# gmweir/PYFFT

Measured on AMD Instinct MI355X. Metric: Msamples/sec Welch-PSD 4096-pt Hann 50% overlap, complex64, higher is better.
Workload: dtype f32

## Files before the change

### pyfft_amd/csrc/k_welch_pipe.hip

```cpp
#include "launch.h"
#include <type_traits>
#define SP_PIPE_AHEAD 2
namespace sp {

template <bool CPLX, int SHIFT, int MODE>
__global__ __launch_bounds__(768) void k_welch_pipe(const void *__restrict__ x_in, const float *__restrict__ win,
                                                     int64_t nframes, int64_t fpg, float *__restrict__ trend_in, XfTables tb,
                                                     float *__restrict__ partial, cf *__restrict__ spartial, int64_t x_cs, int gpr) {
    constexpr int N = 4096;
    constexpr bool RP = MODE >= 3 && MODE != 8 && MODE != 9;
    constexpr bool ONEPASS = MODE == 1 || MODE == 4 || MODE == 7 || MODE == 8 || MODE == 9, COG = MODE == 2 || MODE == 8;
    constexpr bool LOBE = MODE == 9;
    constexpr bool SPEC = MODE == 5 || MODE == 7;
    const void *x = SPEC ? (const void *)(reinterpret_cast<const float *>(x_in) + (int64_t)blockIdx.y * x_cs) : x_in;
    float *trend = SPEC ? trend_in + 4 * blockIdx.y : trend_in;
    static_assert(!RP || (!CPLX && SHIFT == 8), "the real-pair form is for real input at hop = nfft / 2");
    using PL = FftPlan<N>;
    using F = WgFft<N>;
    constexpr int T = PL::T, R = PL::R, KEEP = R - SHIFT, IMG = F::IMG0, IMGB = PL::LDS_ELEMS;
    static_assert(T == 256 && R == 16 && PL::NP == 3, "three radix-16 passes over 256 threads");
    extern __shared__ __attribute__((aligned(16))) unsigned char smem_raw[];
    cf *smem = reinterpret_cast<cf *>(smem_raw);
    cf *imgA = smem, *imgB = smem + 2 * IMG;
    const int role = __builtin_amdgcn_readfirstlane((int)threadIdx.x >> 8);
    const int tid = (int)threadIdx.x & 255;
    const int hop = SHIFT * T;

    cf mu;
    if constexpr (ONEPASS) {
        const int64_t span = (nframes - 1) * (int64_t)hop + N;
        const int64_t pitch = span / 16;
        constexpr int NU = SPEC ? 4 : 1, NTH = SPEC ? 3 * T : T, NWV = SPEC ? 12 : 4;
        const int lt = SPEC ? (int)threadIdx.x : tid;
        float sx = 0.f, sy = 0.f;
#pragma unroll
        for (int r = 0; r < 16; ++r)
#pragma unroll
            for (int u = 0; u < NU; ++u) {
                int64_t i = pitch * r + (int64_t)(lt + NTH * u);
                i = i < span ? i : span - 1;
                const cf v = load_sample(x, i, CPLX);
                sx += v.x;
                sy += v.y;
            }
        sx = wave_sum64(sx);
        sy = wave_sum64(sy);
        float *red = reinterpret_cast<float *>(smem);
        if ((SPEC || role == 0) && (tid & 63) == 0) {
            red[2 * (lt >> 6)] = sx;
            red[2 * (lt >> 6) + 1] = sy;
        }
        __syncthreads();
        double tx = 0.0, ty = 0.0;
#pragma unroll
        for (int wv = 0; wv < NWV; ++wv) {
            tx += (double)red[2 * wv];
            ty += (double)red[2 * wv + 1];
        }
        mu = mk((float)(tx / (16.0 * NTH * NU)), (float)(ty / (16.0 * NTH * NU)));
        __syncthreads();
        if (blockIdx.x == 0 && threadIdx.x == 0) {
            trend[0] = mu.x;
            trend[1] = mu.y;
            trend[2] = 0.f;
            trend[3] = 0.f;
        }
    } else {
        mu = load_trend(trend).m;
    }
    const int64_t gid = blockIdx.x;
    const int64_t g0 = gid * fpg;
    const int64_t last = nframes - 1;
    int64_t trips = (RP ? (nframes + 1) / 2 : nframes) - g0;
    trips = trips < 0 ? 0 : (trips > fpg ? fpg : trips);
    constexpr int DRAIN = 4;
    const int64_t periods = trips + DRAIN;
    F f;
    constexpr bool UPROT = !RP;
    float tau_out[16];
    if constexpr (UPROT) {
        if (role == 0) f.template load_tau_out<0>(tb.tw, tid, tau_out);
        else if (role == 1) f.template load_tau_out<1>(tb.tw, tid, tau_out);
    }

    if (role == 0 && RP) {
        const float *xr = reinterpret_cast<const float *>(x);
        float m = mu.x;
        asm volatile("" : "+v"(m));
        float w[R], sacc[SHIFT];
#pragma unroll
        for (int t = 0; t < R; ++t) w[t] = win[tid + T * t];
#pragma unroll
        for (int s = 0; s < SHIFT; ++s) sacc[s] = 0.f;
        auto issue_chunk = [&](float (&dst)[R], int64_t q) __attribute__((always_inline)) {
            const int64_t q1 = 2 * q <= nframes ? q : 0, q2 = 2 * q + 1 <= nframes ? q : 0;
            const float *b1 = xr + q1 * (int64_t)N, *b2 = xr + q2 * (int64_t)N;
#pragma unroll
            for (int t = 0; t < R; ++t) {
                const unsigned off = (unsigned)(tid + T * t);
                dst[t] = __builtin_nontemporal_load((t < R / 2 ? b1 : b2) + off);
            }
        };
        float ca[R], cb[R], cc[R];
        issue_chunk(ca, g0);
        issue_chunk(cb, g0 + 1);
#pragma unroll
        for (int t = 0; t < R; ++t) {
            ca[t] -= m;
            cb[t] -= m;
        }
        auto frame = [&](auto hb, int64_t i, cf *img, float (&cur)[R], float (&nxt)[R], float (&fill)[R]) __attribute__((always_inline)) {
            constexpr bool HB = decltype(hb)::value;
            issue_chunk(fill, g0 + i + 2);
            __builtin_amdgcn_sched_barrier(0);
            cf v[R];
            if constexpr (!ONEPASS) {
#pragma unroll
                for (int t = 0; t < R; ++t) v[t] = mk(cur[t], HB ? (t < R / 2 ? cur[t + R / 2] : nxt[t - R / 2]) : 0.f);
                if constexpr (UPROT) f.bfly_scatter_win_rot(v, w, tau_out, img, tid);
                else f.bfly_scatter_win(v, w, img, tid);
            } else {
#pragma unroll
                for (int t = 0; t < R; ++t) v[t] = mk(w[t] * cur[t], HB ? w[t] * (t < R / 2 ? cur[t + R / 2] : nxt[t - R / 2]) : 0.f);
                if constexpr (UPROT) f.template bfly_scatter_rot<0, false>(v, tau_out, img, tid);
                else f.template bfly_scatter<0>(v, img, tid);
            }
            __builtin_amdgcn_sched_barrier(0);
            if constexpr (ONEPASS) {
#pragma unroll
                for (int s = 0; s < SHIFT; ++s) sacc[s] += HB ? cur[R / 2 + s] + nxt[s] : cur[R / 2 + s];
            }
#pragma unroll
            for (int t = 0; t < R; ++t) fill[t] -= m;
        };
        const std::true_type yes;
        const std::false_type no;
        int64_t i = 0;
        for (; i + 6 < trips; i += 6) {
            frame(yes, i, imgA, ca, cb, cc);
            __syncthreads();
            frame(yes, i + 1, imgA + IMG, cb, cc, ca);
            __syncthreads();
            frame(yes, i + 2, imgA, cc, ca, cb);
            __syncthreads();
            frame(yes, i + 3, imgA + IMG, ca, cb, cc);
            __syncthreads();
            frame(yes, i + 4, imgA, cb, cc, ca);
            __syncthreads();
            frame(yes, i + 5, imgA + IMG, cc, ca, cb);
            __syncthreads();
        }
        for (; i < trips; ++i) {
            cf *img = (i & 1) ? imgA + IMG : imgA;
            const bool has_b = 2 * (g0 + i) + 1 < nframes;
            if (has_b) {
                if (i % 3 == 0) frame(yes, i, img, ca, cb, cc);
                else if (i % 3 == 1) frame(yes, i, img, cb, cc, ca);
                else frame(yes, i, img, cc, ca, cb);
            } else {
                if (i % 3 == 0) frame(no, i, img, ca, cb, cc);
                else if (i % 3 == 1) frame(no, i, img, cb, cc, ca);
                else frame(no, i, img, cc, ca, cb);
            }
            __syncthreads();
        }
#pragma unroll
        for (int d = 0; d < DRAIN; ++d) __syncthreads();
        if constexpr (ONEPASS) {
#pragma unroll
            for (int s = 0; s < SHIFT; ++s)
                spartial[((SPEC ? (int64_t)blockIdx.y * gridDim.x : 0) + gid) * hop + tid + T * s] = mk(sacc[s], 0.f);
        }
    } else if (role == 0) {
        asm volatile("" : "+v"(mu.x), "+v"(mu.y));
        float w[R];
        cf sacc[SHIFT], raw[R];
#pragma unroll
        for (int t = 0; t < R; ++t) w[t] = win[tid + T * t];
#pragma unroll
        for (int s = 0; s < SHIFT; ++s) sacc[s] = mk(0.f, 0.f);
        {
            const int64_t base = (g0 < nframes ? g0 : last) * hop + tid;
#pragma unroll
            for (int t = 0; t < R; ++t) raw[t] = load_sample(x, base + T * t, CPLX) - mu;
        }
        auto issue_part = [&](cf (&dst)[SHIFT], int64_t q, int s0, int s1) __attribute__((always_inline)) {
            const int64_t gq = g0 + q;
            const int64_t gn = gq < nframes ? gq : last;
            const int64_t ubase = gn * hop + (int64_t)T * KEEP;
#pragma unroll
            for (int s = s0; s < s1; ++s) {
                const unsigned off = (unsigned)(tid + T * s);
                if (CPLX) {
                    const sp_f2v r = __builtin_nontemporal_load(reinterpret_cast<const sp_f2v *>(x) + ubase + off);
                    dst[s] = mk(r.x, r.y);
                } else {
                    dst[s] = mk(__builtin_nontemporal_load(reinterpret_cast<const float *>(x) + ubase + off), 0.f);
                }
            }
        };
        auto issue = [&](cf (&dst)[SHIFT], int64_t q) __attribute__((always_inline)) { issue_part(dst, q, 0, SHIFT); };
        constexpr int AHEAD = (SP_PIPE_AHEAD >= 2 && SHIFT <= 8) ? (SP_PIPE_AHEAD >= 3 ? 3 : 2) : 1;
        constexpr bool SPREAD = AHEAD >= 2;
        auto frame = [&](int64_t i, cf *img, cf (&fill)[SHIFT], cf (&take)[SHIFT]) __attribute__((always_inline)) {
            if constexpr (SPREAD) issue_part(fill, i + AHEAD, 0, SHIFT / 4);
            else issue(fill, i + AHEAD);
            __builtin_amdgcn_sched_barrier(0);
            cf v[R];
            constexpr bool WINFOLD = SPREAD;
#pragma unroll
            for (int t = 0; t < R; ++t) v[t] = WINFOLD ? raw[t] : w[t] * raw[t];
            if constexpr (SPREAD) {
            {
                auto store = [&](int k, cf val) __attribute__((always_inline)) {
                    img[F::template phys<0>(tid * 16 + k)] = UPROT ? rot_tan(val, tau_out[k]) : val;
                    if (k >= 12 && k < 15) issue_part(fill, i + AHEAD, (k - 11) * (SHIFT / 4), (k - 10) * (SHIFT / 4));
                };
                if constexpr (WINFOLD) dft16s_es_win(v, w, store);
                else dft16s_es<false>(v, f.t16[0], store);
            }
            } else {
            if constexpr (UPROT) f.template bfly_scatter_rot<0, false>(v, tau_out, img, tid);
            else f.template bfly_scatter<0>(v, img, tid);
            }
            __builtin_amdgcn_sched_barrier(0);
#pragma unroll
            for (int s = 0; s < SHIFT; ++s)
                if constexpr (ONEPASS && !LOBE) sacc[s] = sacc[s] + raw[KEEP + s];
#pragma unroll
            for (int t = 0; t < KEEP; ++t) raw[t] = raw[t + SHIFT];
#pragma unroll
            for (int s = 0; s < SHIFT; ++s) raw[KEEP + s] = take[s] - mu;
        };
        int64_t i = 0;
        if constexpr (AHEAD == 3) {
            cf s0[SHIFT], s1[SHIFT], s2[SHIFT];
            issue(s1, 1);
            issue(s2, 2);
            for (; i + 2 < trips; i += 3) {
                frame(i, (i & 1) ? imgA + IMG : imgA, s0, s1);
                __syncthreads();
                frame(i + 1, ((i + 1) & 1) ? imgA + IMG : imgA, s1, s2);
                __syncthreads();
                frame(i + 2, ((i + 2) & 1) ? imgA + IMG : imgA, s2, s0);
                __syncthreads();
            }
            for (; i < trips; ++i) {
                cf *img = (i & 1) ? imgA + IMG : imgA;
                if (i % 3 == 0) frame(i, img, s0, s1);
                else if (i % 3 == 1) frame(i, img, s1, s2);
                else frame(i, img, s2, s0);
                __syncthreads();
            }
        } else if constexpr (AHEAD == 2) {
            cf nxa[SHIFT], nxb[SHIFT];
            issue(nxa, 1);
            for (; i + 1 < trips; i += 2) {
                frame(i, imgA, nxb, nxa);
                __syncthreads();
                frame(i + 1, imgA + IMG, nxa, nxb);
                __syncthreads();
            }
            if (i < trips) {
                frame(i, imgA, nxb, nxa);
                __syncthreads();
            }
        } else {
            for (; i + 1 < trips; i += 2) {
                cf nx0[SHIFT], nx1[SHIFT];
                frame(i, imgA, nx0, nx0);
                __syncthreads();
                frame(i + 1, imgA + IMG, nx1, nx1);
                __syncthreads();
            }
            if (i < trips) {
                cf nx0[SHIFT];
                frame(i, imgA, nx0, nx0);
                __syncthreads();
            }
        }
#pragma unroll
        for (int d = 0; d < DRAIN; ++d) __syncthreads();
#pragma unroll
        for (int s = 0; s < SHIFT; ++s)
            if constexpr (ONEPASS && !LOBE) spartial[gid * hop + tid + T * s] = sacc[s];
    } else if (role == 1) {
        f.template load_tw_one<1>(tb.tw, tid);
        cf va[R], vb[R];
        auto step = [&](auto steady, cf (&fill)[R], cf (&use)[R], int64_t p, const cf *src, cf *dst) __attribute__((always_inline)) {
            constexpr bool STEADY = decltype(steady)::value;
            if (STEADY || (p >= 1 && p <= trips)) f.template gather<0>(fill, src, tid);
            if (STEADY || (p >= 2 && p <= trips + 1)) {
                if constexpr (UPROT) f.template bfly_scatter_rot<1, true>(use, tau_out, dst, tid);
                else f.template bfly_scatter<1>(use, dst, tid);
            }
            __syncthreads();
            if constexpr (STEADY) __builtin_amdgcn_sched_barrier(0);
        };
        const std::true_type yes;
        const std::false_type no;
        step(no, va, vb, 0, imgA + IMG, imgB);
        step(no, vb, va, 1, imgA, imgB + IMGB);
        int64_t p = 2;
        for (; p + 1 <= trips; p += 2) {
            step(yes, va, vb, p, imgA + IMG, imgB);
            step(yes, vb, va, p + 1, imgA, imgB + IMGB);
        }
        for (; p < periods; p += 2) {
            step(no, va, vb, p, imgA + IMG, imgB);
            if (p + 1 < periods) step(no, vb, va, p + 1, imgA, imgB + IMGB);
        }
    } else {
        f.template load_tw_one<2>(tb.tw, tid);
        float acc[R];
#pragma unroll
        for (int t = 0; t < R; ++t) acc[t] = 0.f;
        cf bs_lo = mk(0.f, 0.f), bs_hi = mk(0.f, 0.f);
        const unsigned zlo = (unsigned)((tid >> 3) * 512 + (tid & 7));
        cf held[SPEC ? R : 1];
        cf va[R], vb[R];
        cf pend = mk(0.f, 0.f);
        auto flush = [&](int64_t i) __attribute__((always_inline)) {
            const int sel = (int)(i & 63), li = tid & 63;
            const int64_t gg = g0 + (i - sel) + li;
            if (li <= sel && gg < nframes) reinterpret_cast<cf *>(partial)[(int64_t)(tid >> 6) * nframes + gg] = pend;
        };
        auto step = [&](auto steady, cf (&fill)[R], cf (&use)[R], int64_t p, const cf *src) __attribute__((always_inline)) {
            constexpr bool STEADY = decltype(steady)::value;
            if (STEADY || (p >= 3 && p <= trips + 2)) {
                f.template gather<1>(fill, src, tid);
            }
            if (STEADY || (p >= 4 && p <= trips + 3)) {
                if constexpr (UPROT) f.template bfly_prerot<2>(use, tid);
                else f.template bfly<2>(use, tid);
                if constexpr (SPEC) {
                    const int64_t pr = g0 + (p - 4);
                    const bool lone = (pr & 1) == 0 && p == trips + 3;
                    if ((pr & 1) == 0 && !lone) {
#pragma unroll
                        for (int t = 0; t < R; ++t) held[t] = use[t];
                    } else {
                        float4 *zb = reinterpret_cast<float4 *>(partial) + ((pr >> 1) * (int64_t)gpr * 512 + (int64_t)blockIdx.y * 8);
                        unsigned bl = zlo;
                        asm volatile("" : "+v"(bl));
#pragma unroll
                        for (int t = 0; t < R; ++t) {
                            const float4 q = lone ? make_float4(use[t].x, use[t].y, 0.f, 0.f)
                                                  : make_float4(held[t].x, held[t].y, use[t].x, use[t].y);
                            st_stream(zb + (bl + 16384u * t), q);
                        }
                    }
                } else if constexpr (COG) {
                    if constexpr (MODE == 8) {
                        const int64_t gf = g0 + (p - 4);
                        cf *lobe = reinterpret_cast<cf *>(partial) + 4 * nframes + gf * 8;
                        if (gf < nframes) {
                            if (tid <= 3) lobe[3 + tid] = use[0];
                            if (tid >= T - 3) lobe[3 - (T - tid)] = use[R - 1];
                        }
                    }
                    float numc = 0.f, den = 0.f;
#pragma unroll
                    for (int t = 0; t < R; ++t) {
                        const float pw = cnorm(use[t]);
                        numc = fmaf(pw, (float)(T * t - (t >= R / 2 ? N : 0)), numc);
                        den += pw;
                    }
                    float num = fmaf((float)tid, den, numc);
                    num = wave_sum64(num);
                    den = wave_sum64(den);
                    const int64_t i = p - 4;
                    if ((tid & 63) == (int)(i & 63)) pend = mk(num, den);
                    if ((i & 63) == 63 || i == trips - 1) flush(i);
                } else {
#pragma unroll
                    for (int t = 0; t < R; ++t) acc[t] = fmaf(use[t].y, use[t].y, fmaf(use[t].x, use[t].x, acc[t]));
                    if constexpr (LOBE) {
                        bs_lo = bs_lo + use[0];
                        bs_hi = bs_hi + use[R - 1];
                    }
                }
            }
            __syncthreads();
            if constexpr (STEADY) __builtin_amdgcn_sched_barrier(0);
        };
        const std::true_type yes;
        const std::false_type no;
        int64_t p = 0;
#pragma unroll 1
        for (; p < DRAIN; p += 2) {
            step(no, va, vb, p, imgB + IMGB);
            step(no, vb, va, p + 1, imgB);
        }
        for (; p + 1 <= trips + 2; p += 2) {
            step(yes, va, vb, p, imgB + IMGB);
            step(yes, vb, va, p + 1, imgB);
        }
        for (; p < periods; p += 2) {
            step(no, va, vb, p, imgB + IMGB);
            if (p + 1 < periods) step(no, vb, va, p + 1, imgB);
        }
        if constexpr (!COG && !SPEC) {
#pragma unroll
            for (int t = 0; t < R; ++t) partial[gid * N + tid + T * t] = acc[t];
            if constexpr (LOBE) {
                if (tid <= 3) spartial[gid * 8 + 3 + tid] = bs_lo;
                if (tid >= T - 3) spartial[gid * 8 + 3 - (T - tid)] = bs_hi;
                if (tid == 4) spartial[gid * 8 + 7] = mk(0.f, 0.f);
            }
        }
    }
}

bool welch_pipe_eligible(const Xf &xf, int hop) {
    return !xf.blue && xf.L == 4096 && (hop == 2048 || hop == 1024 || hop == 4096);
}

int launch_welch_pipe(LaunchCtx c, const void *x, bool cplx, const float *win, int hop, int64_t nframes, float *trend,
                      const Xf &xf, float *partial, const RunPart &rp, cf *spartial, int mode, int nch, int64_t x_cs, int gpr) {
    const size_t lds = sizeof(cf) * 4 * (size_t)FftPlan<4096>::LDS_ELEMS;
#define PIPE_(CP, S, OP)                                                                                  \
    {                                                                                                 \
        if (lds_raise<k_welch_pipe<CP, S, OP>>(lds)) return -1;                                       \
        if (c.stop)                                                                                   \
            hipExtLaunchKernelGGL((k_welch_pipe<CP, S, OP>), dim3(rp.blocks, gy), dim3(768), lds, c.stream, nullptr, c.stop, 0, x, win, \
                                  nframes, rp.fpg, trend, xf.tb, partial, spartial, x_cs, gpr);       \
        else                                                                                          \
            hipLaunchKernelGGL((k_welch_pipe<CP, S, OP>), dim3(rp.blocks, gy), dim3(768), lds, c.stream, x, win, nframes, rp.fpg, trend, \
                               xf.tb, partial, spartial, x_cs, gpr);                                  \
    }
    const int shift = hop / 256;
    const unsigned gy = mode == 5 ? (unsigned)nch : 1u;
#define PIPE_S_(CP, OP)                                                                               \
    if (shift == 8) PIPE_(CP, 8, OP) else if (shift == 4) PIPE_(CP, 4, OP) else PIPE_(CP, 16, OP)
    if (mode == 5) {
        if (cplx || shift != 8 || nch < 1 || gpr < 1) return -1;
        if (spartial) PIPE_(false, 8, 7) else PIPE_(false, 8, 5)
    } else if (mode == 3) {
        if (cplx || shift != 8) return -1;
        if (spartial) PIPE_(false, 8, 4) else PIPE_(false, 8, 3)
    } else if (mode == 2 && spartial) {
        if (shift == 8) { if (cplx) PIPE_(true, 8, 8) else PIPE_(false, 8, 8) }
        else if (shift == 4) { if (cplx) PIPE_(true, 4, 8) else PIPE_(false, 4, 8) }
        else return -1;
    } else if (mode == 2) {
        if (cplx) { PIPE_S_(true, 2) } else { PIPE_S_(false, 2) }
    } else if (mode == 9) {
        if (!spartial || shift == 16) return -1;
        if (shift == 8) { if (cplx) PIPE_(true, 8, 9) else PIPE_(false, 8, 9) }
        else { if (cplx) PIPE_(true, 4, 9) else PIPE_(false, 4, 9) }
    } else if (spartial) {
        if (cplx) { PIPE_S_(true, 1) } else { PIPE_S_(false, 1) }
    } else {
        if (cplx) { PIPE_S_(true, 0) } else { PIPE_S_(false, 0) }
    }
#undef PIPE_S_
#undef PIPE_
    return 0;
}

}
```

### pyfft_amd/csrc/launch.h

```cpp
#pragma once
#include <limits.h>
#include <stdlib.h>
#include "kernels.h"
#include "nufft_plan.h"
#include "ar_plan.h"
#include "sub_plan.h"
#include "dwt_plan.h"
#include <hip/hip_runtime.h>
#include <hip/hip_ext.h>

namespace sp {

inline bool env_flag(const char *name) {
    const char *v = getenv(name);
    return v && v[0] && v[0] != '0';
}
inline int env_int(const char *name, int dflt) {
    const char *v = getenv(name);
    return v ? atoi(v) : dflt;
}

struct LaunchCtx {
    hipStream_t stream;
    int ncu;
    hipEvent_t stop = nullptr;
};

struct Xf {
    XfTables tb;
    int L;
    bool blue;
};

constexpr int fpw_of(int L) {
    const int R = L < 16 ? L : 16, T = L / R, WG = T >= 256 ? T : 256;
    return WG / T;
}
constexpr size_t xf_image_bytes(int L, int nbuf = 1) { return (size_t)fpw_of(L) * (size_t)(L + 16) * 8 * nbuf; }
template <int L> constexpr bool xf_image_agrees() {
    if constexpr (L < 8192) {
        if (!xf_image_agrees<2 * L>()) return false;
    }
    return WgCfg<L>::FPW == fpw_of(L) && WgCfg<L>::lds_bytes(1) == xf_image_bytes(L) && WgCfg<L>::lds_bytes(2) == xf_image_bytes(L, 2);
}
static_assert(xf_image_agrees<32>(), "fpw_of and xf_image_bytes are the kernels' FPW and lds_bytes at every L of 32 .. 8192");

#define SP_LDS_MAX ((size_t)160 * 1024)
template <auto K> int lds_raise(size_t lds_bytes) {
    static size_t raised = 64 * 1024;
    if (lds_bytes <= raised) return 0;
    if (lds_bytes > SP_LDS_MAX ||
        hipFuncSetAttribute((const void *)K, hipFuncAttributeMaxDynamicSharedMemorySize, (int)SP_LDS_MAX) != hipSuccess)
        return -1;
    raised = SP_LDS_MAX;
    return 0;
}

template <class X> struct XfTag {
    using type = X;
};
template <int LO, int HI, class F> int for_pow2(int L, F f) {
    if (L == LO) return f(XfTag<XfPow2<LO>>{});
    if constexpr (LO < HI) return for_pow2<2 * LO, HI>(L, f);
    else return -1;
}

inline bool runs_cover(int64_t n, int64_t per, int64_t runs) {
    return runs >= 1 && runs <= 0x7fffffff && (runs - 1) * per < n && runs * per >= n;
}
inline bool band_in_transform(bool cplx, int L, int b0, int nb) {
    return nb >= 1 && b0 >= 0 && b0 < L && nb <= L && (cplx || b0 + nb <= L / 2 + 1);
}

struct RunPart {
    int64_t groups, fpg;
    int blocks;
};
inline RunPart run_partition(int L, int64_t nframes, int ncu, int groups_per_cu = 0) {
    if (groups_per_cu <= 0) groups_per_cu = 4;
    const int fpw = fpw_of(L);
    const int64_t target = (int64_t)ncu * groups_per_cu * fpw;
    int64_t f = (nframes + target - 1) / target;
    if (f < 1) f = 1;
    const int64_t G = (nframes + f - 1) / f;
    RunPart r;
    r.fpg = f;
    r.blocks = (int)((G + fpw - 1) / fpw);
    r.groups = (int64_t)r.blocks * fpw;
    return r;
}
inline RunPart run_partition_2d(int L, int64_t nframes, int ncu, int ny, int64_t slots = 0) {
    const int fpw = fpw_of(L);
    int64_t target = ((int64_t)ncu * 8 + ny - 1) / (ny > 0 ? ny : 1) * fpw;
    if (target < 8 * fpw) target = 8 * fpw;
    int64_t f = (nframes + target - 1) / target;
    if (f < 1) f = 1;
    if (slots > 0 && ny > 0) {
        const int64_t wg = ((nframes + f - 1) / f + fpw - 1) / fpw * ny;
        int64_t rounds = (wg + slots / 2) / slots;
        if (rounds < 1) rounds = 1;
        const int64_t groups = rounds * slots / ny * fpw;
        if (groups >= 1) {
            const int64_t f2 = (nframes + groups - 1) / groups;
            if (f2 >= 1 && f2 <= 4 * f) f = f2;
        }
    }
    const int64_t G = (nframes + f - 1) / f;
    RunPart r;
    r.fpg = f;
    r.blocks = (int)((G + fpw - 1) / fpw);
    r.groups = (int64_t)r.blocks * fpw;
    return r;
}
inline int strided_blocks(int L, int64_t items, int ncu, int per_cu = 4) {
    const int fpw = fpw_of(L);
    int64_t b = (items + fpw - 1) / fpw;
    int64_t cap = (int64_t)ncu * (L >= 4096 ? per_cu : 16);
    if (L == 2048) {
        const int64_t q = b / 4;
        if (q < cap) cap = q > (int64_t)ncu * 2 ? q : (int64_t)ncu * 2;
    }
    if (b > cap) b = cap;
    if (b < 1) b = 1;
    return (int)b;
}

int resident_per_cu(const void *fn, int threads, size_t lds_bytes);
int welch_rp_groups_per_cu(const Xf &xf, bool lin);
int csd_pair_resident(const Xf &xf, bool lin, bool onepass);
int stft_rp_groups_per_cu(const Xf &xf, bool lin, int hop, int sided, int out_power, bool pseg);

int launch_fft_c2c(LaunchCtx c, const cf *in, cf *out, int64_t batch, int inverse, const Xf &xf,
                   BigTw bt = BigTw{nullptr, nullptr, 0, 0});
int launch_fft_cols(LaunchCtx c, const cf *in, cf *out, int64_t ncols, int64_t nouter, int64_t es, int64_t os, int64_t twmul,
                    int conj_in, const Xf &xf, BigTw bt, int64_t hmask_n = 0,
                    ColsIn ci = ColsIn{0, nullptr, nullptr, nullptr, 0}, int tw_outer = 0);
int launch_fft_rows_rev(LaunchCtx c, const cf *in, cf *out, int64_t A, int64_t B, int conj_out, float scale, const Xf &xf,
                        RowsOut ro = RowsOut{nullptr, 0, 0, nullptr});
int launch_transpose_c(LaunchCtx c, const cf *in, cf *out, int64_t rows, int64_t cols, int conj, float scale, int64_t batch = 1);
int launch_pack_real(LaunchCtx c, const float *x, int64_t n_in, const double *mean, int64_t L, cf *out);
int launch_cmul_vec(LaunchCtx c, const cf *a, const cf *b, int64_t n, int conj_out, cf *out, int64_t batch = 1);
int launch_blue_pre(LaunchCtx c, const cf *in, const cf *chirp, int64_t n, int64_t L, int conj_in, cf *out, int64_t batch = 1);
int launch_blue_post(LaunchCtx c, const cf *in, const cf *chirp, int64_t n, int conj_out, float scale, cf *out, int64_t batch = 1,
                     int64_t in_ld = 0);
int launch_hilbert_mask(LaunchCtx c, cf *X, int64_t n);
int launch_xc_pack(LaunchCtx c, const float *x1, const float *x2, int64_t n, int64_t L, const double *mom, cf *z);
int launch_xc_mid(LaunchCtx c, const cf *Z, int64_t L, cf *R);
int launch_xc_mid_half(LaunchCtx c, const cf *Z, int64_t L, BigTw bt, cf *Zp);
int launch_xc_out(LaunchCtx c, const cf *r, int64_t n, int64_t L, const double *mom, float *co);
bool welch_carry_eligible(const Xf &xf, int hop, bool lin);
int launch_welch(LaunchCtx c, const void *x, bool cplx, const float *win, int hop, int64_t nframes, const float *trend,
                 bool lin, const Xf &xf, float *partial, const RunPart &rp, bool allow_carry, cf *spartial,
                 const char **kname, int segmean = 0);
bool welch_pipe_eligible(const Xf &xf, int hop);
int launch_welch_pipe(LaunchCtx c, const void *x, bool cplx, const float *win, int hop, int64_t nframes, float *trend,
                      const Xf &xf, float *partial, const RunPart &rp, cf *spartial, int mode = 0, int nch = 1, int64_t x_cs = 0,
                      int gpr = 0);
int launch_op_estimate(LaunchCtx c, const void *x, bool cplx, int64_t nsig, double *part, float *trend);
int launch_op_reduce(LaunchCtx c, const void *x, bool cplx, const float *trend, const float *partial, const cf *spartial,
                     int64_t G, const Xf &xf, int hop, int64_t nframes, int64_t nmean, OnePass st, double *sum_out);
int launch_op_finish(LaunchCtx c, const void *x, bool cplx, const float *trend, const float *win, OnePass st,
                     const double *mean_in, int64_t nmean, const Xf &xf, int hop, int64_t nframes, cf *cw, const cf *Wf,
                     int sided, double scale, double *out, bool export_state = false);
int launch_op_apply(LaunchCtx c, const double *state, const cf *Wf, int n, int sided, double scale, double *out,
                    const double *mean = nullptr);
int opx_tot_blocks();
int launch_welch_opx(LaunchCtx c, const void *x, bool cplx, bool pair, const float *win, int hop, int64_t nframes,
                     const float *trend, const Xf &xf, const RunPart &rp, float *partial, cf *cpart);
int launch_opx_reduce(LaunchCtx c, const float *partial, const cf *cpart, int64_t G, const Xf &xf, const void *x, bool cplx,
                      const float *trend, int hop, int64_t nframes, int64_t nmean, double *A, double *csum, double *tpart);
int launch_opx_finish(LaunchCtx c, const float *win, const double *A, const double *csum, const double *tpart, const float *trend,
                      int hop, int64_t nframes, int64_t nmean, bool sym, const Xf &xf, double *out);
int launch_op_fused(LaunchCtx c, const void *x, bool cplx, const float *trend, const float *win, const float *partial,
                    const cf *spartial, int64_t G, int n, int hop, int64_t nframes, int64_t nmean, OnePass st, unsigned *ticket,
                    CogLobe lb, const double *mean_in, int sided, double scale, double *out, bool export_state,
                    OpPrev prev = OpPrev{nullptr, nullptr, nullptr, 0, 0.0}, bool light = false, double cola_c = 0.0);
int launch_welch_finish(LaunchCtx c, const float *partial, int64_t G, const Xf &xf, int sided, double scale, double *out,
                        int sym = 0);
int launch_welch_rp(LaunchCtx c, const float *x, const float *win, int hop, int64_t nframes, const float *trend, bool lin,
                    const Xf &xf, float *partial, const RunPart &rp);
int launch_stft_rp(LaunchCtx c, const float *x, const float *win, int hop, int64_t nframes, const float *trend, bool lin,
                   const Xf &xf, const RunPart &rp, int sided, float amp, int out_power, void *out, double *pseg,
                   int nchan = 1, int64_t x_cs = 0, int64_t out_cs = 0, int out_ld = 0);
int launch_csd(LaunchCtx c, const void *x, const void *y, bool cplx, int nch, int64_t y_ld, const float *win, int hop,
               int64_t nframes, const float *trend_x, const float *trend_y, bool lin, const Xf &xf, float *partial,
               const RunPart &rp, int segmean = 0);
int launch_csd_finish(LaunchCtx c, const float *partial, int64_t G, const Xf &xf, int nch, int sided, double scale,
                      double *pxx, double *pyy, double *pxy);
int launch_stft(LaunchCtx c, const void *x, bool cplx, const float *win, int hop, int64_t nframes, const float *trend,
                bool lin, const Xf &xf, const RunPart &rp, int sided, float amp, int out_power, void *out, double *pseg, int segmean = 0,
                cf *cog = nullptr, int klo = 0, int khi = 0);
int launch_cog_finish(LaunchCtx c, const cf *acc, int wpf, int64_t nframes, double df, double *out);
int launch_cog_carry(LaunchCtx c, const void *x, bool cplx, const float *win, int hop, int64_t nframes, const float *trend,
                     const Xf &xf, cf *cog, const RunPart &rp, int klo, int khi);
bool csd_rp_eligible(const Xf &xf);
int launch_csd_rp(LaunchCtx c, const float *x, const float *y, int nch, int64_t y_ld, const float *win, int hop,
                  int64_t nframes, const float *trend_x, const float *trend_y, bool lin, const Xf &xf, float *partial,
                  const RunPart &rp);
int launch_csd_rp_finish(LaunchCtx c, const float *partial, int64_t G, const Xf &xf, int nch, int sided, double scale,
                         double *pxx, double *pyy, double *pxy);
int launch_pairspec(LaunchCtx c, const float *x, const float *win, int hop, int64_t nframes, const float *trend, bool lin,
                    const Xf &xf, const RunPart &rp, cf *Zx);
int launch_csd_pair(LaunchCtx c, const float *y, int nch, int64_t y_ld, const float *win, int hop, int64_t nframes,
                    float *trend_y, bool lin, const Xf &xf, const cf *Zx, float *partial, const RunPart &rp, cf *spartial = nullptr);
int launch_csd_pair_finish(LaunchCtx c, const float *partial, int64_t G, const Xf &xf, int nch, int sided, double scale,
                           double *pyy, double *pxy, const double *st_y = nullptr, const double *st_x = nullptr, const cf *Wf = nullptr,
                           const float *trend_x = nullptr, const float *trend_y = nullptr, int64_t nmean = 0, int64_t M = 0);
#define SP_COLSUM_SLICES 256
int launch_colsum_real(LaunchCtx c, const float *x, const float *trend, int H, int64_t M, cf *out);
int launch_csdm_finish(LaunchCtx c, double *G, int nch, int nb, double scale);
int launch_csdm_transpose_kgc(LaunchCtx c, const cf *Xs, cf *Xt, int nch, int nchp, int64_t m, int64_t mp, int nb);
int launch_csdm_mfma(LaunchCtx c, const cf *Xt, int nch, int nchp, int64_t mp, int nb, double *G);
int launch_csdm_bf16(LaunchCtx c, const cf *Xs, cf *Xt_tail, int nch, int64_t m, int nb, double *G, int ld, int two_pieces = 0, int init = 0);
int launch_csdm_fold(LaunchCtx c, const double *H, double *G, int nch, int n, const double *st = nullptr, const cf *Wf = nullptr,
                     const float *trend = nullptr, int64_t nmean = 0, int64_t M = 0, double scale = 1.0, int init = 0);
int launch_cm_blocksums(LaunchCtx c, const cf *spartial, int nch, int runs, int hop, double *Sl);
int launch_op_finish_channels(LaunchCtx c, const void *x, int64_t x_cs, int nch, const float *trend, const float *win,
                              const double *Sl, const cf *Wf, int hop, int64_t nframes, int64_t nmean, const Xf &xf, double *out,
                              bool cplx = false);
int launch_cog_finish_op(LaunchCtx c, const cf *acc, int wpf, int64_t nframes, double df, double *out, const cf *lobe, CogLobe lb,
                         const double *st, const float *trend, int64_t nmean, int n);
int launch_csdm_fused(LaunchCtx c, const cf *Xs, cf *Xt_tail, int nch, int64_t m, int nb, double *G, int ld = 0);
int launch_hilbert_mid(LaunchCtx c, cf *Z, int64_t M, BigTw bt);
int launch_hilbert_rowsmid(LaunchCtx c, cf *Tm, int64_t A, int64_t B, const Xf &xc, BigTw btN, const cf *tw2c);
int launch_xc_rowsmid(LaunchCtx c, cf *Tm, int64_t A, int64_t B, const Xf &xc, const Xf &xc2, BigTw btL, BigTw btM);
int launch_fft_cols_lag(LaunchCtx c, const cf *in, int64_t ncols, int64_t nouter, int64_t es, int64_t os, const Xf &xf, RowsOut ro);
int launch_fft_cols_inv(LaunchCtx c, const cf *in, cf *out, int64_t ncols, int64_t nouter, int64_t es, int64_t os, int64_t twmul,
                        const Xf &xf, BigTw bt, float scale, const RowsOut *analytic);
int launch_hilbert(LaunchCtx c, const float *x, int64_t n_in, int64_t x_ld, int64_t batch, const Xf &xf, cf *out,
                   const cf *H = nullptr);
int launch_spec_mul(LaunchCtx c, cf *X, const cf *H, int64_t n);
int frame_sum_slices(int ncu, int nch, int nfft, int64_t nframes);
int launch_frame_sum(LaunchCtx c, const void *x, bool cplx, int64_t x_ld, int nch, int nfft, int hop, int64_t nframes,
                     const float *trend, bool lin, double *out, double *part);
int launch_fftfilt(LaunchCtx c, const float *x, int64_t n, int ntaps, const cf *Hs, const Xf &xf, float *y);
int launch_xcorr(LaunchCtx c, const float *x1, const float *x2, int64_t n, const double *mom, const Xf &xf, float *co);
int launch_moments(LaunchCtx c, const void *x, bool cplx, int64_t n, int mode, double *partial_scratch, double *out_d,
// ... 768 lines not shown
```

### pyfft_amd/csrc/spectral.hip

```cpp
#include "../../include/spectral.h"
#include "../../include/spectral_ext.h"
#include "../../include/spectral_tfr.h"
#include "../../include/spectral_quad.h"
#include "../../include/spectral_cyclo.h"
#include "../../include/spectral_uneven.h"
#include "../../include/spectral_wbic.h"
#include "../../include/spectral_fam.h"
#include "../../include/spectral_nufft.h"
#include "../../include/spectral_nufft2.h"
#include "../../include/spectral_ar.h"
#include "../../include/spectral_sub.h"
#include "../../include/spectral_dwt.h"
#include "launch.h"
#include "stage.h"
#include "table_cache.h"

#include <hip/hip_runtime.h>
#include <rccl/rccl.h>
#include <dlfcn.h>
#include <limits.h>
#include <math.h>
#include <stdarg.h>
#include <stdio.h>
#include <stdlib.h>
#include <string.h>

#include <map>
#include <mutex>
#include <string>
#include <vector>

using namespace sp;

#define SP_VERSION 110
#define SP_MAX_WG_FFT 8192
#define SP_MAX_BIG_LOG2 26

namespace {

thread_local std::string g_err;

int fail(const char *fmt, ...) {
    char buf[512];
    va_list ap;
    va_start(ap, fmt);
    vsnprintf(buf, sizeof buf, fmt, ap);
    va_end(ap);
    g_err = buf;
    return -1;
}

#define HIPCHK(expr)                                                                                  \
    do {                                                                                              \
        hipError_t e_ = (expr);                                                                       \
        if (e_ != hipSuccess) return fail("%s failed: %s (%s:%d)", #expr, hipGetErrorString(e_), __FILE__, __LINE__); \
    } while (0)
#define LAUNCHCHK(expr)                                                                               \
    do {                                                                                              \
        if ((expr) != 0) return fail("%s: no kernel instantiated for this transform length (%s:%d)", #expr, __FILE__, __LINE__); \
        HIPCHK(hipGetLastError());                                                                    \
    } while (0)

struct Scratch {
    void *p = nullptr;
    size_t cap = 0;
    int ensure(size_t bytes) {
        if (bytes <= cap) return 0;
        if (p) (void)hipFree(p);
        p = nullptr;
        cap = 0;
        size_t want = bytes + (bytes >> 3) + 4096;
        if (hipMalloc(&p, want) != hipSuccess) return fail("hipMalloc(%zu) failed", want);
        cap = want;
        return 0;
    }
    void release() {
        if (p) (void)hipFree(p);
        p = nullptr;
        cap = 0;
    }
};

struct BlueTab {
    cf *chirp, *bf;
    int L;
};

struct Ctx {
    bool ready = false;
    int device = 0;
    int ncu = 256;
    hipStream_t stream = nullptr;
    std::map<int64_t, cf *> twiddles;
    std::map<int64_t, BlueTab> blue;
    Scratch in0, in1, out0, work, small, trends, onepass, ticket, epi;
    Scratch pend_trend;
    Scratch bigA, bigB, bigT, blueA, blueB, longrec;
    Scratch sosY, sosZ;
    Scratch bsIn, bsS, bsP, bsA;
    Scratch mtS;
    Scratch wbW, wbP, wbA;
    Scratch famZ, famA;
    Scratch nuRec, nuGrid;
    Scratch subPart, subMat;
    Scratch dwtS;
    Scratch arPart, arSmall;
    Scratch cmS, cmT, cmG, cmH, cmO;
    std::map<int64_t, BigTw> bigtw;
    std::map<int64_t, BlueTab> blue_big;
    std::mutex mu;
    bool profile = false, prof_valid = false;
    hipEvent_t ev0 = nullptr, ev1 = nullptr, ev_sw = nullptr;
    const char *last_kernel = "";
} g;

LaunchCtx lc() { return LaunchCtx{g.stream, g.ncu}; }

struct Pending {
    bool valid = false;
    const void *xd = nullptr;
    bool cplx = false;
    int64_t nsig = 0, nframes = 0, nmean = 0;
    int nfft = 0, hop = 0;
    Xf xf;
    const float *win_d = nullptr;
    const cf *Wf = nullptr;
    OnePass st;
    float *trend_f = nullptr;
    cf *cw = nullptr;
    double *sum_d = nullptr;
    double *state = nullptr;
} g_pend;

struct ProfScope {
    bool on;
    hipStream_t st;
    explicit ProfScope(hipStream_t s = nullptr) : on(g.profile), st(s ? s : g.stream) {
        if (on) (void)hipEventRecord(g.ev0, st);
    }
    ~ProfScope() {
        if (on) {
            (void)hipEventRecord(g.ev1, st);
            g.prof_valid = true;
        }
    }
};

int ensure_init() {
    if (g.ready) return 0;
    return sp_init(-1);
}

bool is_pow2(int64_t n) { return n >= 1 && (n & (n - 1)) == 0; }
int64_t next_pow2(int64_t n) {
    int64_t p = 1;
    while (p < n) p <<= 1;
    return p;
}

int get_twiddles(int64_t n, const cf **out) {
    auto it = g.twiddles.find(n);
    if (it != g.twiddles.end()) {
        *out = it->second;
        return 0;
    }
    std::vector<cf> h((size_t)n);
    for (int64_t m = 0; m < n; ++m) {
        const double a = -2.0 * M_PI * (double)m / (double)n;
        h[(size_t)m] = make_float2((float)cos(a), (float)sin(a));
    }
    cf *d = nullptr;
    HIPCHK(hipMalloc((void **)&d, sizeof(cf) * (size_t)n));
    HIPCHK(hipMemcpy(d, h.data(), sizeof(cf) * (size_t)n, hipMemcpyHostToDevice));
    g.twiddles[n] = d;
    *out = d;
    return 0;
}

int get_xf(int64_t n, Xf *xf) {
    if (n < 2) return fail("transform length %lld too short", (long long)n);
    if (is_pow2(n) && n <= SP_MAX_WG_FFT) {
        xf->L = (int)n;
        xf->blue = false;
        xf->tb.n = (int)n;
        xf->tb.chirp = xf->tb.bf = nullptr;
        return get_twiddles(n, &xf->tb.tw);
    }
    int64_t L = next_pow2(2 * n - 1);
    if (L < 16) L = 16;
    if (L > SP_MAX_WG_FFT)
        return fail("transform length %lld not supported yet (powers of two up to %d, other lengths up to %d)",
                    (long long)n, SP_MAX_WG_FFT, SP_MAX_WG_FFT / 2);
    xf->L = (int)L;
    xf->blue = true;
    xf->tb.n = (int)n;
    if (get_twiddles(L, &xf->tb.tw)) return -1;
    auto it = g.blue.find(n);
    if (it == g.blue.end()) {
        std::vector<cf> ch((size_t)n), bw((size_t)L, make_float2(0.f, 0.f));
        for (int64_t m = 0; m < n; ++m) {
            const int64_t q = (m * m) % (2 * n);
            const double a = M_PI * (double)q / (double)n;
            ch[(size_t)m] = make_float2((float)cos(a), (float)-sin(a));
            const cf b = make_float2((float)(cos(a) / (double)L), (float)(sin(a) / (double)L));
            bw[(size_t)m] = b;
            if (m > 0) bw[(size_t)(L - m)] = b;
        }
        BlueTab t;
        t.L = (int)L;
        HIPCHK(hipMalloc((void **)&t.chirp, sizeof(cf) * (size_t)n));
        HIPCHK(hipMalloc((void **)&t.bf, sizeof(cf) * (size_t)L));
        HIPCHK(hipMemcpy(t.chirp, ch.data(), sizeof(cf) * (size_t)n, hipMemcpyHostToDevice));
        HIPCHK(hipMemcpy(t.bf, bw.data(), sizeof(cf) * (size_t)L, hipMemcpyHostToDevice));
        Xf p2;
        if (get_xf(L, &p2)) return -1;
        LAUNCHCHK(launch_fft_c2c(lc(), t.bf, t.bf, 1, 0, p2));
        HIPCHK(hipStreamSynchronize(g.stream));
        g.blue[n] = t;
        it = g.blue.find(n);
    }
    xf->tb.chirp = it->second.chirp;
    xf->tb.bf = it->second.bf;
    return 0;
}

TableCache g_tables;

int g_passes[10] = {0, 0, 0, 0, 0, 0, 0, 0, 0, 0};
inline void note_slices(int64_t n) {
    if (n > g_passes[1]) g_passes[1] = (int)n;
}
inline int64_t hook_cap(const char *name, int64_t v) {
    const int64_t h = env_int(name, 0);
    return h > 0 && h < v ? h : v;
}

struct ApiLock {
    std::lock_guard<std::mutex> lk;
    ApiLock() : lk(g.mu) {
        g_tables.begin_call();
        g_passes[0] = g_passes[1] = g_passes[2] = g_passes[3] = g_passes[4] = g_passes[5] = g_passes[6] = g_passes[7] = g_passes[8] = g_passes[9] = 0;
    }
};

struct Stage {
    const bool host;
    int done = 0;
    StagePlan plan;
    explicit Stage(int mem) : host(!mem) {}
    template <class H, class D> void in(Scratch &s, const H *h, size_t bytes, const D **dev) {
        *dev = (const D *)h;
        if (host) plan.add(&s, h, nullptr, bytes, dev);
    }
    template <class H, class D> void out(Scratch &s, H *h, size_t bytes, D **dev) {
        *dev = (D *)h;
        if (host) plan.add(&s, nullptr, h, bytes, dev);
    }
    template <class H, class D> void inout(Scratch &s, const H *h_in, H *h_out, size_t bytes, const D **din, D **dout) {
        *din = (const D *)h_in;
        *dout = (D *)h_out;
        if (host) plan.add(&s, h_in, h_out, bytes, dout, din);
    }
    int commit() {
        if (!host) return 0;
        if (plan.err) return fail("staging: %s", plan.err);
        for (int a = 0; a < plan.nareas; ++a)
            if (!plan.area[a].sealed) {
                if (((Scratch *)plan.area[a].key)->ensure(plan.area[a].total)) return -1;
                plan.seal(a);
// ... 889 lines not shown
    geng.epi = nullptr;
    geng.nsub = 0;
}

int engine_apply_locked(int s) {
    EngineSlot &sl = geng.slot[s];
    const int nfft = (int)sl.win.size();
    Xf xf;
    if (get_xf(nfft, &xf)) return -1;
    void *Wf_d;
    if (get_window_spectrum(sl.win.data(), nfft, xf, &Wf_d)) return -1;
    LAUNCHCHK(launch_op_apply(LaunchCtx{geng.epi, g.ncu}, (const double *)geng.st[s].p, (const cf *)Wf_d, nfft, sl.sided,
                              sl.scale / (double)sl.frames_total, sl.out));
    return 0;
}

bool welch_generic_shape(int nfft, int hop) {
    if (!wg_capable(nfft)) return false;
    Xf xf;
    if (get_xf(nfft, &xf)) return false;
    return !welch_carry_eligible(xf, hop, false);
}

int welch_export_locked(const void *xd, bool cplx, int64_t nsig, const float *win, int nfft, int hop, int64_t nframes,
                        int64_t nmean, double *st_d, const OpPrev *prev = nullptr, hipEvent_t prev_wait = nullptr,
                        bool *prev_done = nullptr, const SplitLaunch *sl = nullptr) {
    FusedOut fo{true, SP_SIDED_RAW, 1.0, st_d, false};
    if (prev) {
        fo.prev = *prev;
        fo.prev_wait = prev_wait;
    }
    if (welch_accum_locked(xd, cplx, nsig, win, nfft, hop, nframes, nmean, false, &fo, sl)) return -1;
    g_pend.valid = false;
    if (prev_done) *prev_done = fo.prev_done;
    if (fo.done) return 0;
    LAUNCHCHK(launch_op_finish(sl ? LaunchCtx{sl->epi, g.ncu} : lc(), g_pend.xd, g_pend.cplx, g_pend.trend_f, g_pend.win_d, g_pend.st, nullptr, g_pend.nmean,
                               g_pend.xf, g_pend.hop, g_pend.nframes, g_pend.cw, g_pend.Wf, SP_SIDED_RAW, 1.0, st_d, true));
    return 0;
}

}

extern "C" {

int sp_version(void) { return SP_VERSION; }
int sp_max_wg_fft(void) { return SP_MAX_WG_FFT; }
const char *sp_last_error(void) { return g_err.c_str(); }
int sp_last_passes(int which) {
    std::lock_guard<std::mutex> lk(g.mu);
    return which >= 0 && which <= 9 ? g_passes[which] : 0;
}

int sp_init(int device_id) {
    std::lock_guard<std::mutex> lk(g.mu);
    if (g.ready && (device_id < 0 || device_id == g.device)) return 0;
    if (g.ready)
        return fail("libspectral is bound to device %d for the life of the process (asked for %d)", g.device, device_id);
    int count = 0;
    if (hipGetDeviceCount(&count) != hipSuccess || count <= 0)
        return fail("no HIP device visible (libspectral has no CPU fallback)");
    if (device_id < 0) {
        if (hipGetDevice(&device_id) != hipSuccess) device_id = 0;
    }
    if (device_id >= count) return fail("device %d out of range (%d visible)", device_id, count);
    HIPCHK(hipSetDevice(device_id));
    hipDeviceProp_t prop;
    HIPCHK(hipGetDeviceProperties(&prop, device_id));
    if (strncmp(prop.gcnArchName, "gfx950", 6) != 0)
        return fail("device %d is %s; libspectral is built for gfx950 only", device_id, prop.gcnArchName);
    g.device = device_id;
    g.ncu = prop.multiProcessorCount > 0 ? prop.multiProcessorCount : 256;
    g.ready = true;
    return 0;
}

void sp_shutdown(void) {
    (void)sp_comm_destroy();
    std::lock_guard<std::mutex> lk(g.mu);
    if (!g.ready) return;
    engine_release();
    (void)hipDeviceSynchronize();
    for (auto &kv : g.twiddles) (void)hipFree(kv.second);
    g.twiddles.clear();
    for (auto &kv : g.blue) {
        (void)hipFree(kv.second.chirp);
        (void)hipFree(kv.second.bf);
    }
    g.blue.clear();
    g.in0.release();
    g.in1.release();
    g.out0.release();
    g.work.release();
    g.small.release();
    g.trends.release();
    g.onepass.release();
    g.ticket.release();
    g.epi.release();
    g.pend_trend.release();
    g.cmS.release();
    g.cmT.release();
    g.cmG.release();
    g.cmH.release();
    g.cmO.release();
    g.bigA.release();
    g.bigB.release();
    g.bigT.release();
    g.blueA.release();
    g.blueB.release();
    g.longrec.release();
    g.mtS.release();
    g.wbW.release();
    g.wbP.release();
    g.wbA.release();
    g.famZ.release();
    g.famA.release();
    g.nuRec.release();
    g.nuGrid.release();
    g.arPart.release();
    g.subPart.release();
    g.subMat.release();
    g.dwtS.release();
    g.arSmall.release();
    for (auto &kv : g.bigtw) {
        (void)hipFree((void *)kv.second.hi);
        (void)hipFree((void *)kv.second.lo);
    }
    g.bigtw.clear();
    for (auto &kv : g.blue_big) {
        (void)hipFree(kv.second.chirp);
        (void)hipFree(kv.second.bf);
    }
    g.blue_big.clear();
    czt_release();
    g_cztAcc.release();
    g_pend.valid = false;
    tables_release();
    g.ready = false;
}

int sp_set_stream(void *hip_stream) {
    if (ensure_init()) return -1;
    ApiLock lk;
    hipStream_t ns = (hipStream_t)hip_stream;
    if (ns != g.stream) {
        if (!g.ev_sw && hipEventCreateWithFlags(&g.ev_sw, hipEventDisableTiming) != hipSuccess) g.ev_sw = nullptr;
        if (g.ev_sw) {
            if (hipEventRecord(g.ev_sw, g.stream) == hipSuccess) (void)hipStreamWaitEvent(ns, g.ev_sw, 0);
            (void)hipGetLastError();
        }
        g.stream = ns;
    }
    return 0;
}

int sp_synchronize(void) {
    if (ensure_init()) return -1;
    HIPCHK(hipStreamSynchronize(g.stream));
    return 0;
}

int sp_profile_enable(int on) {
    if (ensure_init()) return -1;
    if (on && !g.ev0) {
        HIPCHK(hipEventCreate(&g.ev0));
        HIPCHK(hipEventCreate(&g.ev1));
    }
// ... 4582 lines not shown
```

Before: 492,200.

## Precompute per-thread FFT twiddle rows and overlap kernel prologue loads

Adds a one-time kernel that packs each thread's tau and radix-16 twiddle values into a coalesced float4 table, which each pipe role loads directly instead of computing from the raw twiddle array. The prologue is also reordered so the one-pass mean-estimation loads, the first-frame loads and the twiddle-row loads are all issued before their values are consumed, and the mean subtraction is deferred until after the prefetch. The goal is to shorten the kernel startup latency. The cost is an extra cached device buffer, a dependency on xf.pipe being set, and more live registers during the prologue.

```diff
diff --git a/pyfft_amd/csrc/k_welch_pipe.hip b/pyfft_amd/csrc/k_welch_pipe.hip
--- a/pyfft_amd/csrc/k_welch_pipe.hip
+++ b/pyfft_amd/csrc/k_welch_pipe.hip
@@ -3,9 +3,51 @@
 #define SP_PIPE_AHEAD 2
 namespace sp {
 
+__global__ __launch_bounds__(PipeConsts::T) void k_pipe_consts(const cf *__restrict__ tw, float4 *__restrict__ out) {
+    using PC = PipeConsts;
+    const int tid = (int)threadIdx.x;
+    WgFft<4096> f;
+    float tau0[16], tau1[16];
+    f.template load_tau_out<0>(tw, tid, tau0);
+    f.template load_tau_out<1>(tw, tid, tau1);
+    f.template load_tw_one<1>(tw, tid);
+    f.template load_tw_one<2>(tw, tid);
+#pragma unroll
+    for (int j = 0; j < 4; ++j) {
+        out[(PC::FRONT_TAU + j) * PC::T + tid] = make_float4(tau0[4 * j], tau0[4 * j + 1], tau0[4 * j + 2], tau0[4 * j + 3]);
+        out[(PC::MID_TAU + j) * PC::T + tid] = make_float4(tau1[4 * j], tau1[4 * j + 1], tau1[4 * j + 2], tau1[4 * j + 3]);
+    }
+#pragma unroll
+    for (int j = 0; j < 10; ++j) {
+        const float *a = f.t16[0].f + 4 * j, *b = f.t16[1].f + 4 * j;
+        out[(PC::MID_TW + j) * PC::T + tid] = make_float4(a[0], a[1], a[2], a[3]);
+        out[(PC::BACK_TW + j) * PC::T + tid] = make_float4(b[0], b[1], b[2], b[3]);
+    }
+}
+
+int launch_pipe_consts(LaunchCtx c, const cf *tw, float4 *out) {
+    hipLaunchKernelGGL(k_pipe_consts, dim3(1), dim3(PipeConsts::T), 0, c.stream, tw, out);
+    return 0;
+}
+
+template <int NQ> __device__ __forceinline__ void pipe_rows_issue(const float4 *__restrict__ pc, int row0, int tid, float4 (&q)[NQ]) {
+#pragma unroll
+    for (int j = 0; j < NQ; ++j) q[j] = pc[(row0 + j) * PipeConsts::T + tid];
+}
+template <int NQ> __device__ __forceinline__ void pipe_rows_take(const float4 (&q)[NQ], float *dst) {
+#pragma unroll
+    for (int j = 0; j < NQ; ++j) {
+        dst[4 * j] = q[j].x;
+        dst[4 * j + 1] = q[j].y;
+        dst[4 * j + 2] = q[j].z;
+        dst[4 * j + 3] = q[j].w;
+        asm volatile("" : "+v"(dst[4 * j]), "+v"(dst[4 * j + 1]), "+v"(dst[4 * j + 2]), "+v"(dst[4 * j + 3]));
+    }
+}
+
 template <bool CPLX, int SHIFT, int MODE>
 __global__ __launch_bounds__(768) void k_welch_pipe(const void *__restrict__ x_in, const float *__restrict__ win,
-                                                     int64_t nframes, int64_t fpg, float *__restrict__ trend_in, XfTables tb,
+                                                     int64_t nframes, int64_t fpg, float *__restrict__ trend_in, const float4 *__restrict__ pc,
                                                      float *__restrict__ partial, cf *__restrict__ spartial, int64_t x_cs, int gpr) {
     constexpr int N = 4096;
     constexpr bool RP = MODE >= 3 && MODE != 8 && MODE != 9;
@@ -26,27 +68,35 @@
     const int tid = (int)threadIdx.x & 255;
     const int hop = SHIFT * T;
 
-    cf mu;
-    if constexpr (ONEPASS) {
+    constexpr int NU = SPEC ? 4 : 1, NTH = SPEC ? 3 * T : T, NWV = SPEC ? 12 : 4;
+    const int lt = SPEC ? (int)threadIdx.x : tid;
+    constexpr bool EARLY = !RP && SHIFT != 16;
+    auto mu0_issue = [&](cf (&mv)[16 * NU]) __attribute__((always_inline)) {
         const int64_t span = (nframes - 1) * (int64_t)hop + N;
         const int64_t pitch = span / 16;
-        constexpr int NU = SPEC ? 4 : 1, NTH = SPEC ? 3 * T : T, NWV = SPEC ? 12 : 4;
-        const int lt = SPEC ? (int)threadIdx.x : tid;
-        float sx = 0.f, sy = 0.f;
 #pragma unroll
         for (int r = 0; r < 16; ++r)
 #pragma unroll
             for (int u = 0; u < NU; ++u) {
                 int64_t i = pitch * r + (int64_t)(lt + NTH * u);
                 i = i < span ? i : span - 1;
-                const cf v = load_sample(x, i, CPLX);
-                sx += v.x;
-                sy += v.y;
-            }
-        sx = wave_sum64(sx);
-        sy = wave_sum64(sy);
+                mv[NU * r + u] = load_sample(x, i, CPLX);
+            }
+        __builtin_amdgcn_sched_barrier(0);
+    };
+    auto mu0_reduce = [&](auto loaded, const cf (&mv)[16 * NU]) __attribute__((always_inline)) {
+        float sx = 0.f, sy = 0.f;
+        if constexpr (decltype(loaded)::value) {
+#pragma unroll
+            for (int k = 0; k < 16 * NU; ++k) {
+                sx += mv[k].x;
+                sy += mv[k].y;
+            }
+            sx = wave_sum64(sx);
+            sy = wave_sum64(sy);
+        }
         float *red = reinterpret_cast<float *>(smem);
-        if ((SPEC || role == 0) && (tid & 63) == 0) {
+        if (decltype(loaded)::value && (tid & 63) == 0) {
             red[2 * (lt >> 6)] = sx;
             red[2 * (lt >> 6) + 1] = sy;
         }
@@ -57,17 +107,36 @@
             tx += (double)red[2 * wv];
             ty += (double)red[2 * wv + 1];
         }
-        mu = mk((float)(tx / (16.0 * NTH * NU)), (float)(ty / (16.0 * NTH * NU)));
+        const cf m = mk((float)(tx / (16.0 * NTH * NU)), (float)(ty / (16.0 * NTH * NU)));
         __syncthreads();
         if (blockIdx.x == 0 && threadIdx.x == 0) {
-            trend[0] = mu.x;
-            trend[1] = mu.y;
+            trend[0] = m.x;
+            trend[1] = m.y;
             trend[2] = 0.f;
             trend[3] = 0.f;
         }
-    } else {
-        mu = load_trend(trend).m;
-    }
+        return m;
+    };
+    auto mu0_other = [&]() __attribute__((always_inline)) {
+        if constexpr (ONEPASS) {
+            cf mv[16 * NU];
+            if constexpr (SPEC) {
+                mu0_issue(mv);
+                (void)mu0_reduce(std::true_type{}, mv);
+            } else {
+                (void)mu0_reduce(std::false_type{}, mv);
+            }
+        }
+    };
+    auto mu_front = [&]() __attribute__((always_inline)) {
+        if constexpr (ONEPASS) {
+            cf mv[16 * NU];
+            mu0_issue(mv);
+            return mu0_reduce(std::true_type{}, mv);
+        } else {
+            return load_trend(trend).m;
+        }
+    };
     const int64_t gid = blockIdx.x;
     const int64_t g0 = gid * fpg;
     const int64_t last = nframes - 1;
@@ -77,17 +146,12 @@
     const int64_t periods = trips + DRAIN;
     F f;
     constexpr bool UPROT = !RP;
-    float tau_out[16];
-    if constexpr (UPROT) {
-        if (role == 0) f.template load_tau_out<0>(tb.tw, tid, tau_out);
-        else if (role == 1) f.template load_tau_out<1>(tb.tw, tid, tau_out);
-    }
 
     if (role == 0 && RP) {
         const float *xr = reinterpret_cast<const float *>(x);
-        float m = mu.x;
+        float m = mu_front().x;
         asm volatile("" : "+v"(m));
-        float w[R], sacc[SHIFT];
+        float w[R], sacc[SHIFT], tau_out[16];
 #pragma unroll
         for (int t = 0; t < R; ++t) w[t] = win[tid + T * t];
 #pragma unroll
@@ -172,9 +236,12 @@
                 spartial[((SPEC ? (int64_t)blockIdx.y * gridDim.x : 0) + gid) * hop + tid + T * s] = mk(sacc[s], 0.f);
         }
     } else if (role == 0) {
-        asm volatile("" : "+v"(mu.x), "+v"(mu.y));
-        float w[R];
+        float w[R], tau_out[16];
         cf sacc[SHIFT], raw[R];
+        float4 qtau[4];
+        if constexpr (UPROT) pipe_rows_issue<4>(pc, PipeConsts::FRONT_TAU, tid, qtau);
+        cf mu = mk(0.f, 0.f);
+        if constexpr (!EARLY) mu = mu_front();
 #pragma unroll
         for (int t = 0; t < R; ++t) w[t] = win[tid + T * t];
 #pragma unroll
@@ -182,7 +249,7 @@
         {
             const int64_t base = (g0 < nframes ? g0 : last) * hop + tid;
 #pragma unroll
-            for (int t = 0; t < R; ++t) raw[t] = load_sample(x, base + T * t, CPLX) - mu;
+            for (int t = 0; t < R; ++t) raw[t] = load_sample(x, base + T * t, CPLX);
         }
         auto issue_part = [&](cf (&dst)[SHIFT], int64_t q, int s0, int s1) __attribute__((always_inline)) {
             const int64_t gq = g0 + q;
@@ -202,6 +269,13 @@
         auto issue = [&](cf (&dst)[SHIFT], int64_t q) __attribute__((always_inline)) { issue_part(dst, q, 0, SHIFT); };
         constexpr int AHEAD = (SP_PIPE_AHEAD >= 2 && SHIFT <= 8) ? (SP_PIPE_AHEAD >= 3 ? 3 : 2) : 1;
         constexpr bool SPREAD = AHEAD >= 2;
+        cf nxa[AHEAD == 2 ? SHIFT : 1], nxb[AHEAD == 2 ? SHIFT : 1];
+        if constexpr (AHEAD == 2) issue(nxa, 1);
+        if constexpr (EARLY) mu = mu_front();
+        if constexpr (UPROT) pipe_rows_take<4>(qtau, tau_out);
+        asm volatile("" : "+v"(mu.x), "+v"(mu.y));
+#pragma unroll
+        for (int t = 0; t < R; ++t) raw[t] = raw[t] - mu;
         auto frame = [&](int64_t i, cf *img, cf (&fill)[SHIFT], cf (&take)[SHIFT]) __attribute__((always_inline)) {
             if constexpr (SPREAD) issue_part(fill, i + AHEAD, 0, SHIFT / 4);
             else issue(fill, i + AHEAD);
@@ -253,8 +327,6 @@
                 __syncthreads();
             }
         } else if constexpr (AHEAD == 2) {
-            cf nxa[SHIFT], nxb[SHIFT];
-            issue(nxa, 1);
             for (; i + 1 < trips; i += 2) {
                 frame(i, imgA, nxb, nxa);
                 __syncthreads();
@@ -285,7 +357,14 @@
         for (int s = 0; s < SHIFT; ++s)
             if constexpr (ONEPASS && !LOBE) spartial[gid * hop + tid + T * s] = sacc[s];
     } else if (role == 1) {
-        f.template load_tw_one<1>(tb.tw, tid);
+        float tau_out[16];
+        float4 qtau[4], qtw[10];
+        if constexpr (SPEC) mu0_other();
+        if constexpr (UPROT) pipe_rows_issue<4>(pc, PipeConsts::MID_TAU, tid, qtau);
+        pipe_rows_issue<10>(pc, PipeConsts::MID_TW, tid, qtw);
+        if constexpr (!SPEC) mu0_other();
+        if constexpr (UPROT) pipe_rows_take<4>(qtau, tau_out);
+        pipe_rows_take<10>(qtw, f.t16[0].f);
         cf va[R], vb[R];
         auto step = [&](auto steady, cf (&fill)[R], cf (&use)[R], int64_t p, const cf *src, cf *dst) __attribute__((always_inline)) {
             constexpr bool STEADY = decltype(steady)::value;
@@ -311,7 +390,11 @@
             if (p + 1 < periods) step(no, vb, va, p + 1, imgA, imgB + IMGB);
         }
     } else {
-        f.template load_tw_one<2>(tb.tw, tid);
+        float4 qtw[10];
+        if constexpr (SPEC) mu0_other();
+        pipe_rows_issue<10>(pc, PipeConsts::BACK_TW, tid, qtw);
+        if constexpr (!SPEC) mu0_other();
+        pipe_rows_take<10>(qtw, f.t16[1].f);
         float acc[R];
 #pragma unroll
         for (int t = 0; t < R; ++t) acc[t] = 0.f;
@@ -419,15 +502,16 @@
 int launch_welch_pipe(LaunchCtx c, const void *x, bool cplx, const float *win, int hop, int64_t nframes, float *trend,
                       const Xf &xf, float *partial, const RunPart &rp, cf *spartial, int mode, int nch, int64_t x_cs, int gpr) {
     const size_t lds = sizeof(cf) * 4 * (size_t)FftPlan<4096>::LDS_ELEMS;
+    if (!xf.pipe) return -1;
 #define PIPE_(CP, S, OP)                                                                                  \
     {                                                                                                 \
         if (lds_raise<k_welch_pipe<CP, S, OP>>(lds)) return -1;                                       \
         if (c.stop)                                                                                   \
             hipExtLaunchKernelGGL((k_welch_pipe<CP, S, OP>), dim3(rp.blocks, gy), dim3(768), lds, c.stream, nullptr, c.stop, 0, x, win, \
-                                  nframes, rp.fpg, trend, xf.tb, partial, spartial, x_cs, gpr);       \
+                                  nframes, rp.fpg, trend, xf.pipe, partial, spartial, x_cs, gpr);     \
         else                                                                                          \
             hipLaunchKernelGGL((k_welch_pipe<CP, S, OP>), dim3(rp.blocks, gy), dim3(768), lds, c.stream, x, win, nframes, rp.fpg, trend, \
-                               xf.tb, partial, spartial, x_cs, gpr);                                  \
+                               xf.pipe, partial, spartial, x_cs, gpr);                                \
     }
     const int shift = hop / 256;
     const unsigned gy = mode == 5 ? (unsigned)nch : 1u;
diff --git a/pyfft_amd/csrc/launch.h b/pyfft_amd/csrc/launch.h
--- a/pyfft_amd/csrc/launch.h
+++ b/pyfft_amd/csrc/launch.h
@@ -30,6 +30,12 @@
     XfTables tb;
     int L;
     bool blue;
+    const float4 *pipe = nullptr;
+};
+
+struct PipeConsts {
+    static constexpr int T = 256, FRONT_TAU = 0, MID_TAU = 4, MID_TW = 8, BACK_TW = 18, ROWS = 28;
+    static constexpr size_t BYTES = sizeof(float4) * ROWS * T;
 };
 
 constexpr int fpw_of(int L) {
@@ -153,6 +159,7 @@
                  bool lin, const Xf &xf, float *partial, const RunPart &rp, bool allow_carry, cf *spartial,
                  const char **kname, int segmean = 0);
 bool welch_pipe_eligible(const Xf &xf, int hop);
+int launch_pipe_consts(LaunchCtx c, const cf *tw, float4 *out);
 int launch_welch_pipe(LaunchCtx c, const void *x, bool cplx, const float *win, int hop, int64_t nframes, float *trend,
                       const Xf &xf, float *partial, const RunPart &rp, cf *spartial, int mode = 0, int nch = 1, int64_t x_cs = 0,
                       int gpr = 0);
diff --git a/pyfft_amd/csrc/spectral.hip b/pyfft_amd/csrc/spectral.hip
--- a/pyfft_amd/csrc/spectral.hip
+++ b/pyfft_amd/csrc/spectral.hip
@@ -93,6 +93,7 @@
     hipStream_t stream = nullptr;
     std::map<int64_t, cf *> twiddles;
     std::map<int64_t, BlueTab> blue;
+    float4 *pipe_consts = nullptr;
     Scratch in0, in1, out0, work, small, trends, onepass, ticket, epi;
     Scratch pend_trend;
     Scratch bigA, bigB, bigT, blueA, blueB, longrec;
@@ -177,14 +178,31 @@
     return 0;
 }
 
+int get_pipe_consts(const cf *tw, const float4 **out) {
+    if (!g.pipe_consts) {
+        float4 *d = nullptr;
+        HIPCHK(hipMalloc((void **)&d, PipeConsts::BYTES));
+        if (launch_pipe_consts(lc(), tw, d) != 0 || hipGetLastError() != hipSuccess) {
+            (void)hipFree(d);
+            return fail("k_pipe_consts: launch failed");
+        }
+        HIPCHK(hipStreamSynchronize(g.stream));
+        g.pipe_consts = d;
+    }
+    *out = g.pipe_consts;
+    return 0;
+}
+
 int get_xf(int64_t n, Xf *xf) {
     if (n < 2) return fail("transform length %lld too short", (long long)n);
+    xf->pipe = nullptr;
     if (is_pow2(n) && n <= SP_MAX_WG_FFT) {
         xf->L = (int)n;
         xf->blue = false;
         xf->tb.n = (int)n;
         xf->tb.chirp = xf->tb.bf = nullptr;
-        return get_twiddles(n, &xf->tb.tw);
+        if (get_twiddles(n, &xf->tb.tw)) return -1;
+        return n == 4096 ? get_pipe_consts(xf->tb.tw, &xf->pipe) : 0;
     }
     int64_t L = next_pow2(2 * n - 1);
     if (L < 16) L = 16;
@@ -1240,6 +1258,8 @@
     (void)hipDeviceSynchronize();
     for (auto &kv : g.twiddles) (void)hipFree(kv.second);
     g.twiddles.clear();
+    if (g.pipe_consts) (void)hipFree(g.pipe_consts);
+    g.pipe_consts = nullptr;
     for (auto &kv : g.blue) {
         (void)hipFree(kv.second.chirp);
         (void)hipFree(kv.second.bf);
```

Result: no change. 492,900, median of 6 (+0.1%).
